# LeCAR-Lab/CoVO-MPC

Hardware: AMD Instinct MI355X
Metric: mpc_control_steps_per_sec (higher is better)
Workload: dtype f32; 1 GPU; covo-online tracking_zigzag N=65536 H=32 lam=0.01 sigma=0.5 (teacher-forced on the recorded inputs -- noisy state, a_mean, key -- of this controller's own 300-step closed-loop episode, timed steps spread evenly over the episode; samples sharded 1x65536, one exchange of the 516-float rank records per step: collective); controller=covo-online, task=tracking_zigzag, N_global=65536, N_local=65536, H=32, pos_stats_info=False

## Files before the change

### covo_mpc_amd/csrc/hessian_adj_body.hpp

```cpp
constexpr int NX = ADJ_NX, NZ = NX + 4, NH = NX + 1, HH = COVO_H, NA = COVO_NA;
constexpr size_t WS_X = 0;
constexpr size_t WS_JF = WS_X + 32 * 16;
constexpr size_t WS_GL = WS_JF + 32 * NX * NZ;
constexpr size_t WS_LAM = WS_GL + 32 * 16;
constexpr size_t WS_MXX = WS_LAM + 33 * 16;
constexpr size_t WS_MXU = WS_MXX + 32 * 256;
constexpr size_t WS_MUU = WS_MXU + 32 * 64;
constexpr size_t WS_S = WS_MUU + 32 * 16;
constexpr int NPAIR = NZ * (NZ + 1) / 2;
constexpr int PAIR_THREADS = (NPAIR + 63) / 64 * 64;
constexpr size_t WS_COUNT = WS_S + (size_t)32 * 16 * NA + 2;
constexpr unsigned long long ADJ_LAM_UNSET = 0xFFF7ADEADBEEF000ull;


__device__ __forceinline__ void adj_force(const float *__restrict__ st, const AdjArgs &A, int bi, int k, double (&f)[3])
{
    if (k == 0) {
        f[0] = st[ST_FDIST + 0]; f[1] = st[ST_FDIST + 1]; f[2] = st[ST_FDIST + 2];
    } else if (A.f_tab != nullptr) {
        const float4 r = A.f_tab[(size_t)bi * HH + k];
        f[0] = r.x; f[1] = r.y; f[2] = r.z;
    } else {
        f[0] = f[1] = f[2] = 0.0;
    }
// ... 363 lines not shown
        const long long t0 = wall_clock64();
        for (;;) {
            bool unset = false;
#pragma unroll
            for (int i = 0; i < NX; ++i) {
                lam[i] = __hip_atomic_load(Lk + i, __ATOMIC_RELAXED, __HIP_MEMORY_SCOPE_AGENT);
                unset |= (unsigned long long)__double_as_longlong(lam[i]) == ADJ_LAM_UNSET;
            }
            if (!unset) break;
            if (wall_clock64() - t0 > 50000000LL) {
                if (A.status != nullptr) __hip_atomic_fetch_or(A.status, COVO_DEVSTAT_ADJOINT, __ATOMIC_RELAXED, __HIP_MEMORY_SCOPE_SYSTEM);
                break;
            }
            __builtin_amdgcn_s_sleep(2);
        }
#pragma unroll
        for (int i = 0; i < NX; ++i) g = fma(lam[i], h[1 + i], g);
    }
    double *__restrict__ Mxx = ws + WS_MXX + (size_t)k * 256, *__restrict__ Mxu = ws + WS_MXU + (size_t)k * 64;
    double *__restrict__ Muu = ws + WS_MUU + (size_t)k * 16;
    if (bb < NX) {
        Mxx[a * 16 + bb] = g;
        Mxx[bb * 16 + a] = g;
    } else if (a < NX) {
        Mxu[a * 4 + (bb - NX)] = g;
    } else {
        Muu[(a - NX) * 4 + (bb - NX)] = g;
        Muu[(bb - NX) * 4 + (a - NX)] = g;
    }
}

__device__ __forceinline__ void adj_hd_padding(const AdjArgs &A, int k, int b, int tid, int nthreads)
{
    double *__restrict__ ws = A.ws + (size_t)b * WS_COUNT;
    double *__restrict__ Mxx = ws + WS_MXX + (size_t)k * 256, *__restrict__ Mxu = ws + WS_MXU + (size_t)k * 64;
    for (int e = tid; e < 256; e += nthreads)
        if ((e >> 4) >= NX || (e & 15) >= NX) Mxx[e] = 0.0;
    if (tid < (16 - NX) * 4) Mxu[NX * 4 + tid] = 0.0;
}

__global__ __launch_bounds__(256) void adj_hd_kernel(const AdjArgs A)
{
    adj_hd_padding(A, (int)blockIdx.x, (int)blockIdx.y, (int)threadIdx.x, 256);
    adj_hd_pairs(A, (int)blockIdx.x, (int)blockIdx.y, (int)threadIdx.x);
}

__global__ __launch_bounds__(256) void adj_chain_kernel(const AdjArgs A)
{
    __shared__ double sjf[(HH - 1) * NX * NZ + 1];
    __shared__ double sgl[HH * 16];
    const int b = blockIdx.y, tid = threadIdx.x, lane = tid & 63, lo = lane & 15, hi = lane >> 4;
    const int w = blockIdx.x;
    double *__restrict__ ws = A.ws + (size_t)b * WS_COUNT;
    if (w >= 9) {
        adj_hd_padding(A, w - 9, b, tid, 256);
        adj_hd_pairs(A, w - 9, b, tid);
        return;
    }
    {
        constexpr int NJ = (HH - 1) * NX * NZ, TJ = (NJ + 255) / 256;
        double vj[TJ];
#pragma unroll
        for (int t = 0; t < TJ; ++t) vj[t] = (tid + 256 * t < NJ) ? ws[WS_JF + tid + 256 * t] : 0.0;
        const double vg0 = ws[WS_GL + tid], vg1 = ws[WS_GL + 256 + tid];
#pragma unroll
        for (int t = 0; t < TJ; ++t)
            if (tid + 256 * t < NJ) sjf[tid + 256 * t] = vj[t];
        sgl[tid] = vg0;
        sgl[256 + tid] = vg1;
        if (tid == 0) sjf[NJ] = 0.0;
    }
    __syncthreads();
    if (tid >= 64) return;
    constexpr int ZI = (HH - 1) * NX * NZ;
    if (w == 8) {
        const double *__restrict__ G = sgl;
        double *__restrict__ L = ws + WS_LAM;
        f64x4 lam;
#pragma unroll
        for (int r = 0; r < 4; ++r) lam[r] = (lo == 0 && hi + 4 * r < NX) ? G[16 * (HH - 1) + hi + 4 * r] : 0.0;
        if (lo == 0) {
#pragma unroll
            for (int r = 0; r < 4; ++r) {
                __hip_atomic_store(&L[16 * (HH - 1) + hi + 4 * r], lam[r], __ATOMIC_RELAXED, __HIP_MEMORY_SCOPE_AGENT);
                __hip_atomic_store(&L[16 * HH + hi + 4 * r], 0.0, __ATOMIC_RELAXED, __HIP_MEMORY_SCOPE_AGENT);
            }
        }
        int offA[4];
        bool okA[4];
#pragma unroll
        for (int g = 0; g < 4; ++g) {
            okA[g] = lo < NX && 4 * g + hi < NX;
            offA[g] = (4 * g + hi) * NZ + lo;
        }
        bool okG[4];
#pragma unroll
        for (int r = 0; r < 4; ++r) okG[r] = lo == 0 && hi + 4 * r < NX;
        double an[4];
        f64x4 gn;
#pragma unroll
        for (int g = 0; g < 4; ++g) an[g] = sjf[okA[g] ? (HH - 2) * NX * NZ + offA[g] : ZI];
#pragma unroll
        for (int r = 0; r < 4; ++r) gn[r] = okG[r] ? G[16 * (HH - 2) + hi + 4 * r] : 0.0;
#pragma unroll
        for (int k = HH - 2; k >= 1; --k) {
            double ac[4];
            f64x4 acc = gn;
#pragma unroll
            for (int g = 0; g < 4; ++g) ac[g] = an[g];
            if (k > 1) {
#pragma unroll
                for (int g = 0; g < 4; ++g) an[g] = sjf[okA[g] ? (k - 1) * NX * NZ + offA[g] : ZI];
#pragma unroll
                for (int r = 0; r < 4; ++r) gn[r] = okG[r] ? G[16 * (k - 1) + hi + 4 * r] : 0.0;
            }
#pragma unroll
            for (int g = 0; g < 4; ++g) acc = __builtin_amdgcn_mfma_f64_16x16x4f64(ac[g], lam[g], acc, 0, 0, 0);
            lam = acc;
            if (lo == 0) {
#pragma unroll
                for (int r = 0; r < 4; ++r) __hip_atomic_store(&L[16 * k + hi + 4 * r], lam[r], __ATOMIC_RELAXED, __HIP_MEMORY_SCOPE_AGENT);
            }
        }
        return;
    }
    const int col = 16 * w + lo, tcol = col >> 2, dcol = col & 3, k0 = 4 * w;
    double *__restrict__ S = ws + WS_S;
    for (int k = 0; k <= k0; ++k) {
#pragma unroll
        for (int r = 0; r < 4; ++r) S[((size_t)k * 16 + hi + 4 * r) * NA + col] = 0.0;
    }
    f64x4 sv = {0.0, 0.0, 0.0, 0.0};
    int offA[4];
    bool okA[4];
#pragma unroll
    for (int g = 0; g < 4; ++g) {
        okA[g] = lo < NX && 4 * g + hi < NX;
        offA[g] = lo * NZ + 4 * g + hi;
    }
    double an[4];
    f64x4 bn;
#pragma unroll
    for (int g = 0; g < 4; ++g) an[g] = sjf[okA[g] ? k0 * NX * NZ + offA[g] : ZI];
#pragma unroll
    for (int r = 0; r < 4; ++r) bn[r] = (tcol == k0 && hi + 4 * r < NX) ? sjf[(k0 * NX + hi + 4 * r) * NZ + NX + dcol] : 0.0;
    double *__restrict__ Sp = S + (size_t)hi * NA + col;
#pragma unroll
    for (int k = 0; k < HH - 1; ++k) {
        if (k < k0) continue;
        double ac[4];
        f64x4 acc = bn;
#pragma unroll
        for (int g = 0; g < 4; ++g) ac[g] = an[g];
        if (k + 1 < HH - 1) {
#pragma unroll
            for (int g = 0; g < 4; ++g) an[g] = sjf[okA[g] ? (k + 1) * NX * NZ + offA[g] : ZI];
            if (k + 1 <= k0 + 3) {
#pragma unroll
                for (int r = 0; r < 4; ++r)
                    bn[r] = (tcol == k + 1 && hi + 4 * r < NX) ? sjf[((k + 1) * NX + hi + 4 * r) * NZ + NX + dcol] : 0.0;
            } else {
#pragma unroll
                for (int r = 0; r < 4; ++r) bn[r] = 0.0;
            }
        }
#pragma unroll
        for (int g = 0; g < 4; ++g) acc = __builtin_amdgcn_mfma_f64_16x16x4f64(ac[g], sv[g], acc, 0, 0, 0);
        sv = acc;
#pragma unroll
        for (int r = 0; r < 4; ++r) Sp[((size_t)(k + 1) * 16 + 4 * r) * NA] = sv[r];
    }
}

__device__ __forceinline__ void adj_tri_tile(int w, int &ti, int &tj)
{
    ti = 0;
    while ((ti + 1) * (ti + 2) / 2 <= w) ++ti;
    tj = w - ti * (ti + 1) / 2;
}

__global__ __launch_bounds__(512) void adj_gemm_kernel(const AdjArgs A)
{
    __shared__ double red[8][4][64];
    __shared__ double sMu[4][64];
    __shared__ double sMuu[64];
    const int b = blockIdx.y, tid = threadIdx.x, lane = tid & 63, wv = tid >> 6, lo = lane & 15, hi = lane >> 4;
    const double *__restrict__ ws = A.ws + (size_t)b * WS_COUNT;
    double *__restrict__ R = A.R + (size_t)b * NA * NA;
    int I, J;
    adj_tri_tile(blockIdx.x, I, J);
    const double *__restrict__ S = ws + WS_S, *__restrict__ Mxx = ws + WS_MXX;
    f64x4 acc = {0.0, 0.0, 0.0, 0.0};
#ifdef KD_PROF
    const long long kp0 = clock64();
#endif
    double ma[4][4], sj[4][4], si[4][4];
#pragma unroll
    for (int it = 0; it < 4; ++it) {
        const int k = 4 * I + 1 + wv + 8 * it;
        const bool on = k < HH;
        const double *__restrict__ Sk = S + (size_t)(on ? k : 0) * 16 * NA, *__restrict__ Mk = Mxx + (size_t)(on ? k : 0) * 256;
        const double2 *__restrict__ Mk2 = reinterpret_cast<const double2 *>(Mk + lo * 16 + 4 * hi);
        const double2 m01 = on ? Mk2[0] : make_double2(0.0, 0.0), m23 = on ? Mk2[1] : make_double2(0.0, 0.0);
        ma[it][0] = m01.x;
        ma[it][1] = m01.y;
        ma[it][2] = m23.x;
        ma[it][3] = m23.y;
#pragma unroll
        for (int g = 0; g < 4; ++g) {
            sj[it][g] = on ? Sk[(size_t)(4 * hi + g) * NA + 16 * J + lo] : 0.0;
            si[it][g] = on ? Sk[(size_t)(4 * g + hi) * NA + 16 * I + lo] : 0.0;
        }
    }
    const int i = 16 * I + hi + 4 * (wv & 3), j = 16 * J + lo;
    const int ti = i >> 2, di = i & 3, tj = j >> 2, dj = j & 3;
    const int tk = ti > tj ? ti : tj, dk = ti > tj ? di : dj;
    double es[NX];
    if (wv < 4) {
        const int col = ti > tj ? j : i;
        const double *__restrict__ Sk = S + (size_t)tk * 16 * NA;
#pragma unroll
        for (int m = 0; m < NX; ++m) es[m] = Sk[(size_t)m * NA + col];
    } else if (wv == 4) {
        sMuu[lane] = ws[WS_MUU + (size_t)(4 * I) * 16 + lane];
    }
// ... 61 lines not shown
```

### covo_mpc_amd/csrc/reduce.hip

```cpp
#include <cstdlib>
#include <cstring>
#include "covo_common.hpp"
#include "softmax_merge.hpp"
#include "softmax_stage1.hpp"

__global__ __launch_bounds__(256) void groupmin_kernel(const float *__restrict__ cost, int N, float *__restrict__ gm)
{
    const int n = blockIdx.x * 256 + threadIdx.x;
    const float wm = wave_min(n < N ? cost[n] : __builtin_inff());
    if ((threadIdx.x & 63) == 0 && (n >> 6) < (N + 63) / 64) gm[n >> 6] = wm;
}


template <bool COV>
__global__ __launch_bounds__(RD_BLOCK) void softmax_partial_kernel(const float *__restrict__ cost,
                                                                   const float4 *__restrict__ a, int N,
                                                                   const float *__restrict__ blockmin, int nbm,
                                                                   float inv_lam, float *__restrict__ partials,
                                                                   const float4 *__restrict__ mu)
{
    softmax_partial_body<COV, false>(cost, a, N, SoftmaxWeights{blockmin, nbm, inv_lam}, partials, mu, nullptr);
}
template <bool COV>
__global__ __launch_bounds__(RD_BLOCK) void softmax_partial_diag_kernel(const float *__restrict__ cost,
                                                                        const float4 *__restrict__ a, int N,
                                                                        const float *__restrict__ blockmin, int nbm,
                                                                        float inv_lam, float *__restrict__ partials,
                                                                        const float4 *__restrict__ mu, float *__restrict__ dpart)
{
    softmax_partial_body<COV, true>(cost, a, N, SoftmaxWeights{blockmin, nbm, inv_lam}, partials, mu, dpart);
}


template <bool FINAL, bool INST = false>
__global__ __launch_bounds__(MG_THREADS) void merge_cov_kernel(const float *__restrict__ partials, int G, float inv_lam,
                                                               const float *__restrict__ a_mean_old, float gamma_mean,
                                                               const float *__restrict__ a_cov_old, float gamma_sigma,
                                                               float *__restrict__ a_mean_out, float *__restrict__ a_cov_out,
                                                               int stride, float *__restrict__ iter_out, int iter_stride)
{
    if (INST) {
        const size_t x = blockIdx.x;
        partials += x * G * stride;
        a_mean_old += x * COVO_NA;
        a_cov_old += x * (COVO_H * 16);
        a_mean_out += x * COVO_NA;
        a_cov_out += x * (COVO_H * 16);
        if (iter_out != nullptr) iter_out += x * (size_t)iter_stride;
    }
    merge_cov_body<FINAL>(partials, G, inv_lam, a_mean_old, gamma_mean, a_cov_old, gamma_sigma, a_mean_out, a_cov_out, stride, iter_out);
}

template <bool FINAL>
__global__ __launch_bounds__(MG_THREADS) void merge_kernel(const float *__restrict__ partials, int G, float inv_lam,
                                                           const float *__restrict__ a_mean_old, float gamma_mean,
                                                           float *__restrict__ out, int stride, float *__restrict__ iter_out,
                                                           int iter_stride)
{
    merge_instance<FINAL, false>(partials, G, inv_lam, a_mean_old, gamma_mean, out, stride, nullptr, nullptr, 0.0f, iter_out, iter_stride);
}

template <bool FINAL>
__global__ __launch_bounds__(MG_THREADS) void merge_diag_kernel(const float *__restrict__ partials, int G, float inv_lam,
                                                                const float *__restrict__ a_mean_old, float gamma_mean,
                                                                float *__restrict__ out, int stride, const float *__restrict__ dpart,
                                                                float *__restrict__ diag_out, float n_samples, float *__restrict__ iter_out,
                                                                int iter_stride)
{
    merge_instance<FINAL, true>(partials, G, inv_lam, a_mean_old, gamma_mean, out, stride, dpart, diag_out, n_samples, iter_out, iter_stride);
}

__global__ void diag_log_rows_kernel(const float *__restrict__ diag, float *__restrict__ log, int n_inst, int stride, int index)
{
    const int i = blockIdx.x * blockDim.x + threadIdx.x;
    if (i < n_inst * COVO_DIAG_FLOATS) {
        const int e = i / COVO_DIAG_FLOATS, j = i % COVO_DIAG_FLOATS;
        log[((size_t)e * stride + index) * COVO_DIAG_FLOATS + j] = diag[i];
    }
}

int launch_diag_log_rows(const float *diag, float *log, int n_inst, int stride, int index, hipStream_t s)
{
    const int n = n_inst * COVO_DIAG_FLOATS;
    hipLaunchKernelGGL(diag_log_rows_kernel, dim3((n + 255) / 256), dim3(256), 0, s, diag, log, n_inst, stride, index);
    COVO_CHECK_HIP(hipGetLastError());
    return 0;
}

__global__ void shift_mean_kernel(const float *__restrict__ in, float *__restrict__ out)
{
    const int i = threadIdx.x;
    out[i] = (i < COVO_NA - COVO_DU) ? in[i + COVO_DU] : in[i];
}

struct Minima {
    const float *blockmin;
    int n_blockmin;
};
static Minima stage1_minima(covo_ctx *h, const UpdateDesc &d, hipStream_t s)
{
    if (d.blockmin != nullptr) return {d.blockmin, d.n_blockmin};
    hipLaunchKernelGGL(groupmin_kernel, dim3((d.N + 255) / 256), dim3(256), 0, s, d.cost, d.N, h->ws_blockmin);
    return {h->ws_blockmin, (d.N + 63) / 64};
}

int launch_softmax_reduce(covo_ctx *h, const UpdateDesc &d, hipStream_t s)
{
    if (d.lam_rows != nullptr) return launch_softmax_reduce_lam(h, d, s);
    const float inv_lam = 1.0f / h->cfg.lam;
    float *partials_ws = d.partials_ws ? d.partials_ws : h->ws_partials;
    const Minima mn = stage1_minima(h, d, s);
    const int grid = stage1_grid(h, d.N);
// ... 97 lines not shown
```

### covo_mpc_amd/csrc/sigma_ns.hip

```cpp
#include "covo_common.hpp"
#include <cstdlib>
#include <cstring>
#include "wave_reduce.hpp"
#include "chol_lds.hpp"
#include "eps_tiles.hpp"
#include "sym_stats.hpp"
#include "noise_gemm_body.hpp"

typedef double f64x4 __attribute__((ext_vector_type(4)));

#ifdef NS_EVAL_STAMPS
#define EV_STAMP(s, i) do { if (threadIdx.x == 0) (s)[SC_STAMPS + 96 + (i)] = (double)wall_clock64(); } while (0)
#else
#define EV_STAMP(s, i) do { } while (0)
#endif
#define EV_STAMP8(s, k, i) do { if ((k) == 8) EV_STAMP(s, 70 + (i)); } while (0)
constexpr int SN = COVO_NA;
constexpr int NS_SQUARINGS = 16;
constexpr double NS_CUT_MARGIN = 1.0 / 1024.0;
constexpr double NS_SQ_TOL = 1e-7;
constexpr double NS_SQ_TGUARD = 1e10;
constexpr int NS_ITERS = 12;
constexpr double NS_TOL2 = 1e-8;
constexpr int RITZ = 4;
// ... 1343 lines not shown
__global__ __launch_bounds__(256) void ns_iter_tail_pair_kernel(const double *A, const NsBufs B, double *scall, int batch, int force_agent)
{
    extern __shared__ __attribute__((aligned(16))) double ld_sm[];
    ns_iter_tail_pair_impl<EARLY_LOGDET>(A, B, scall, batch, force_agent, 0, ld_sm);
}
template <int NEVAL>
__global__ __launch_bounds__(256) void ns_chain_kernel(const double *A, const XBufs xb_all, const NsBufs B, double *scall, int force_agent,
                                                       int deflate)
{
    extern __shared__ __attribute__((aligned(16))) double ld_sm[];
    static_assert(NS_SQ_DYN_DOUBLES * sizeof(double) <= (size_t)SN * (SN + 1) * sizeof(double), "the squaring side's LDS fits the launch's");
    static_assert(NS_SQ_PAIR_WG + NEVAL <= NS_PAIR_WG, "grid = 8 x NS_PAIR_WG covers the squaring side");
    if ((blockIdx.x & 7u) == 0u) {
        ns_square_tail_pair_impl<NEVAL, false, true>(A, xb_all, scall, 1, force_agent, deflate, ld_sm);
        return;
    }
    ns_iter_tail_pair_impl<true>(A, B, scall, 1, force_agent, 1, ld_sm);
}

template <int NWAVES>
__device__ void ns_logdetB_workgroup(const double *__restrict__ A, double *__restrict__ s, double *__restrict__ sm, double *__restrict__ red)
{
    constexpr int THREADS = 64 * NWAVES, LD = SN + 1;
    const int tid = threadIdx.x;
    const double delta = s[SC_DELTA];
    const double2 *A2 = reinterpret_cast<const double2 *>(A);
#pragma unroll 4
    for (int e = tid; e < SN * SN / 2; e += THREADS) {
        const int r = e / (SN / 2), c = 2 * (e % (SN / 2));
        const double2 v = A2[e];
        sm[c * LD + r] = v.x + ((r == c) ? delta : 0.0);
        sm[(c + 1) * LD + r] = v.y + ((r == c + 1) ? delta : 0.0);
    }
    __syncthreads();
    chol128_lds_mfma<LD, NWAVES>(sm, tid);
    if (tid < SN) {
        const double d = sm[tid * LD + tid];
        const double pm = wr::wave64_allprod(__builtin_amdgcn_frexp_mant(d));
        const double pe = wr::wave64_allsum((double)__builtin_amdgcn_frexp_exp(d));
        if ((tid & 63) == 0) {
            red[2 * (tid >> 6)] = pm;
            red[2 * (tid >> 6) + 1] = pe;
        }
    }
    __syncthreads();
    if (tid == 0) {
        const double sumlog = fma(red[1] + red[3], 0.6931471805599453, log(red[0] * red[2]));
        gst<COH_AGENT>(s + SC_SUMLOGB, sumlog);
        asm volatile("s_waitcnt vmcnt(0)" ::: "memory");
        gst<COH_AGENT>(s + SC_LDFLAG, 1.0);
    }
}

__global__ __launch_bounds__(512) void ns_finalize_kernel(const double *__restrict__ Z0all, const double *__restrict__ Z1all,
                                                          const double *__restrict__ Zt0all, const double *__restrict__ Zt1all,
                                                          double *__restrict__ scall, float sample_sigma,
                                                          float *__restrict__ Sigma_out, float *__restrict__ L_out, int batch,
                                                          const EpsGenArgs gen, int *status, const double *__restrict__ Aall,
                                                          int logdet_here)
{
    extern __shared__ __attribute__((aligned(16))) double sm[];
    __shared__ double red[512];
    if (logdet_here && (int)blockIdx.x < 2 * batch && ((int)blockIdx.x & 1) == 0) {
        const int b = (int)blockIdx.x >> 1;
        ns_logdetB_workgroup<8>(Aall + (size_t)b * SN * SN, scall + (size_t)b * SC_COUNT, sm, red);
        return;
    }
    const int first_passenger = logdet_here ? 2 * batch : batch;
    if ((int)blockIdx.x >= first_passenger) {
        eps_tiles_generate(gen, ((int)blockIdx.x - first_passenger) * 8 + (int)(threadIdx.x >> 6), ((int)gridDim.x - first_passenger) * 8,
                           (int)(threadIdx.x & 63));
        return;
    }
    const int b = logdet_here ? (int)blockIdx.x >> 1 : (int)blockIdx.x, tid = threadIdx.x;
    double *s = scall + (size_t)b * SC_COUNT;
    __shared__ double suv[SN];
    const double uv_mine = (tid < SN) ? s[SC_U + tid] : 0.0;
    const bool z1 = s[SC_ZBUF] != 0.0;
    const double zc = s[SC_ZCOEF];
    if (tid < SN) suv[tid] = uv_mine;
    const double *uv = suv;
    const double2 *Z = reinterpret_cast<const double2 *>((z1 ? Z1all : Z0all) + (size_t)b * SN * SN);
    const double2 *Zt = reinterpret_cast<const double2 *>((z1 ? Zt1all : Zt0all) + (size_t)b * SN * SN);
    constexpr int LD = SN + 1;
    const double n = (double)SN;
    long long tk[5];
    tk[0] = clock64();
    {
        constexpr int TR = NS_TILES * 128 / 512;
        double2 za[TR], zt[TR];
#pragma unroll
        for (int t = 0; t < TR; ++t) {
            const int w = __builtin_amdgcn_readfirstlane((tid >> 7) + 4 * t), in = tid & 127;
            int ti, tj;
            tri_tile(w, ti, tj);
            const int e2 = ((16 * ti + (in >> 3)) * SN + 16 * tj + 2 * (in & 7)) >> 1;
            za[t] = Z[e2];
            zt[t] = Zt[e2];
        }
        __syncthreads();
#pragma unroll
        for (int t = 0; t < TR; ++t) {
            const int w = __builtin_amdgcn_readfirstlane((tid >> 7) + 4 * t), in = tid & 127;
            int ti, tj;
            tri_tile(w, ti, tj);
            const int r = 16 * ti + (in >> 3), c = 16 * tj + 2 * (in & 7);
            double v0 = 0.5 * (za[t].x + zt[t].x), v1 = 0.5 * (za[t].y + zt[t].y);
            if (zc != 0.0) {
                const double ur = zc * uv[r];
                v0 = fma(ur, uv[c], v0);
                v1 = fma(ur, uv[c + 1], v1);
            }
            sm[c * LD + r] = v0;
            sm[(c + 1) * LD + r] = v1;
            if (ti == tj) {
                sm[r * LD + c] = v0;
                sm[r * LD + c + 1] = v1;
            }
        }
    }
    __syncthreads();
    tk[1] = clock64();
    chol128_lds_mfma<LD>(sm, tid);
    tk[2] = clock64();
    if (tid == 0) {
        const long long t0 = wall_clock64();
        int good = 1;
        while (gld<COH_AGENT>(s + SC_LDFLAG) == 0.0) {
            __builtin_amdgcn_s_sleep(1);
            if (wall_clock64() - t0 > 20000000LL) {
                good = 0;
                break;
            }
        }
        red[0] = gld<COH_AGENT>(s + SC_SUMLOGB);
        red[1] = good ? 0.0 : 1.0;
    }
    __syncthreads();
    const double sumlogB = red[0];
    const bool ld_failed = red[1] != 0.0;
    const double poison = (s[SC_BARFAIL] != 0.0 || ld_failed) ? __builtin_nan("") : 1.0;
    if (tid == 0 && (s[SC_BARFAIL] != 0.0 || ld_failed) && status != nullptr)
        __hip_atomic_fetch_or(status, COVO_DEVSTAT_GRID_BARRIER, __ATOMIC_RELAXED, __HIP_MEMORY_SCOPE_SYSTEM);
    const double cz = poison * ((double)sample_sigma * (double)sample_sigma) * exp(sumlogB / n) * qm::rsq64_(s[SC_SCALE]);
    const double sq = cz * qm::rsq64_(cz);
    if (tid == 0) s[SC_CZ] = cz;
    tk[3] = clock64();
    constexpr int TRS = SN * SN / 2 / 512;
    double2 za[TRS], zt[TRS];
    if (Sigma_out) {
#pragma unroll
        for (int t = 0; t < TRS; ++t) {
            za[t] = Z[tid + 512 * t];
            zt[t] = Zt[tid + 512 * t];
        }
    }
    float *Lo = L_out + (size_t)b * SN * SN;
#pragma unroll 4
    for (int e = tid; e < SN * SN; e += 512) {
        const int r = e / SN, c = e % SN;
        Lo[e] = (c <= r) ? (float)(sq * sm[c * LD + r]) : 0.0f;
    }
    if (Sigma_out) {
        float2 *So = reinterpret_cast<float2 *>(Sigma_out + (size_t)b * SN * SN);
#pragma unroll
        for (int t = 0; t < TRS; ++t) {
            const int e = 2 * (tid + 512 * t), r = e / SN, c = e % SN;
            double v0 = 0.5 * (za[t].x + zt[t].x), v1 = 0.5 * (za[t].y + zt[t].y);
            if (zc != 0.0) {
                const double ur = zc * uv[r];
                v0 = fma(ur, uv[c], v0);
                v1 = fma(ur, uv[c + 1], v1);
            }
            So[tid + 512 * t] = make_float2((float)(cz * v0), (float)(cz * v1));
        }
    }
    tk[4] = clock64();
    if (tid == 0) {
        for (int i = 0; i < 5; ++i) s[SC_PROF + i] = (double)(tk[i] - tk[0]);
    }
}


struct StreamHook {
    const double *sm;
    double sq;
    float *Lg;
    unsigned *sync;
    unsigned seq;
    int *cnt;
    double *stamps;
    int tid;
    static constexpr int LD = SN + 1;
    __device__ __forceinline__ void panel_done(int p) const
    {
        const int wave = tid >> 6, lane = tid & 63;
#ifdef NS_STREAM_STAMPS
        if (tid == 0) stamps[2 + p] = (double)wall_clock64();
#endif
        if (wave == 0) return;
        const int rr = lane >> 4, kk = lane & 15, j0 = 16 * p, c = j0 + kk;
        for (int i0 = j0 + 4 * (wave - 1); i0 < SN; i0 += 28) {
            const int i = i0 + rr;
            const float v = (c <= i) ? (float)(sq * sm[c * LD + i]) : 0.0f;
            __hip_atomic_store(Lg + (size_t)i * SN + c, v, __ATOMIC_RELAXED, __HIP_MEMORY_SCOPE_AGENT);
        }
    }
    __device__ __forceinline__ void before_barrier(int p) const
    {
        const int wave = tid >> 6, lane = tid & 63;
        if (p == 0 || wave == 0) return;
        asm volatile("s_waitcnt vmcnt(0)" ::: "memory");
        if (lane == 0) {
            const int old = __hip_atomic_fetch_add(cnt + (p - 1), 1, __ATOMIC_RELAXED, __HIP_MEMORY_SCOPE_WORKGROUP);
            if (old == 6) {
                __hip_atomic_store(sync + p, seq, __ATOMIC_RELAXED, __HIP_MEMORY_SCOPE_AGENT);
#ifdef NS_STREAM_STAMPS
                stamps[11 + (p - 1)] = (double)wall_clock64();
#endif
            }
        }
    }
};

template <int P>
__device__ __forceinline__ bool stream_wait_panel(const StreamGemmArgs &S, unsigned seq, int *flag_lds)
{
    if (threadIdx.x == 0) {
        const long long t0 = wall_clock64();
        int good = 1;
        while (__hip_atomic_load(S.sync + 1 + P, __ATOMIC_RELAXED, __HIP_MEMORY_SCOPE_AGENT) != seq) {
            __builtin_amdgcn_s_sleep(1);
            if (wall_clock64() - t0 > 20000000LL) {
                good = 0;
                break;
            }
        }
        *flag_lds = good;
    }
    __syncthreads();
    return *flag_lds != 0;
}
template <int P>
__device__ __forceinline__ void stream_stage_panel(const float *__restrict__ L, float *__restrict__ Ls, int tid)
{
    constexpr int R0 = 32 * (P / 2), CHUNKS = (COVO_NA - R0) * 4;
    if (tid < CHUNKS) {
        const int i = R0 + (tid >> 2), k4 = 16 * P + 4 * (tid & 3);
        const unsigned long long *src = reinterpret_cast<const unsigned long long *>(L + (size_t)i * COVO_NA + k4);
        const unsigned long long lo = __hip_atomic_load(src, __ATOMIC_RELAXED, __HIP_MEMORY_SCOPE_AGENT);
        const unsigned long long hi = __hip_atomic_load(src + 1, __ATOMIC_RELAXED, __HIP_MEMORY_SCOPE_AGENT);
        float *d = Ls + i * NG_LDA + k4;
        d[0] = (k4 + 0 <= i) ? __uint_as_float((unsigned)lo) : 0.0f;
        d[1] = (k4 + 1 <= i) ? __uint_as_float((unsigned)(lo >> 32)) : 0.0f;
        d[2] = (k4 + 2 <= i) ? __uint_as_float((unsigned)hi) : 0.0f;
        d[3] = (k4 + 3 <= i) ? __uint_as_float((unsigned)(hi >> 32)) : 0.0f;
    }
}
__global__ __launch_bounds__(512) void ns_finalize_stream_kernel(const double *__restrict__ Z0, const double *__restrict__ Z1,
                                                                 const double *__restrict__ Zt0, const double *__restrict__ Zt1,
                                                                 double *__restrict__ s, float sample_sigma, const StreamGemmArgs S,
                                                                 int *status)
{
    extern __shared__ __attribute__((aligned(16))) double sm[];
    __shared__ double red[8];
    __shared__ int flag_lds;
    const int tid = threadIdx.x, lane = tid & 63;
    const int wave = __builtin_amdgcn_readfirstlane(tid >> 6);
    constexpr int LD = SN + 1;
    const double n = (double)SN;
    if (tid == 0) {
        const long long t0 = wall_clock64();
        int good = 1;
        while (gld<COH_AGENT>(s + SC_LDFLAG) == 0.0) {
            __builtin_amdgcn_s_sleep(1);
            if (wall_clock64() - t0 > 20000000LL) {
                good = 0;
                break;
            }
        }
        red[0] = gld<COH_AGENT>(s + SC_SUMLOGB);
        red[1] = good ? 0.0 : 1.0;
    }
    __syncthreads();
    const double sumlogB = red[0];
    const bool bad = s[SC_BARFAIL] != 0.0 || red[1] != 0.0;
    const double poison = bad ? __builtin_nan("") : 1.0;
    const double cz = poison * ((double)sample_sigma * (double)sample_sigma) * exp(sumlogB / n) * qm::rsq64_(s[SC_SCALE]);
    const double sq = cz * qm::rsq64_(cz);
    const unsigned seq = __hip_atomic_load(S.sync, __ATOMIC_RELAXED, __HIP_MEMORY_SCOPE_AGENT);
    const bool z1 = s[SC_ZBUF] != 0.0;
    const double zc = s[SC_ZCOEF];
#ifdef NS_STREAM_STAMPS
    double *stamps = s + SC_STAMPS;
#define STREAM_STAMP(i) do { if (tid == 0) stamps[(i)] = (double)wall_clock64(); } while (0)
#else
#define STREAM_STAMP(i) do { } while (0)
#endif

    if (blockIdx.x == 0) {
        STREAM_STAMP(0);
        if (tid == 0 && bad && status != nullptr)
            __hip_atomic_fetch_or(status, COVO_DEVSTAT_GRID_BARRIER, __ATOMIC_RELAXED, __HIP_MEMORY_SCOPE_SYSTEM);
        if (tid == 0) s[SC_CZ] = cz;
        __shared__ double suv[SN];
        __shared__ int wcnt[8];
        if (tid < SN) suv[tid] = s[SC_U + tid];
        if (tid < 8) wcnt[tid] = 0;
        const double2 *Z = reinterpret_cast<const double2 *>(z1 ? Z1 : Z0);
        const double2 *Zt = reinterpret_cast<const double2 *>(z1 ? Zt1 : Zt0);
        long long tk[3];
        tk[0] = clock64();
        {
            constexpr int TR = NS_TILES * 128 / 512;
            double2 za[TR], zt[TR];
#pragma unroll
            for (int t = 0; t < TR; ++t) {
                const int w = __builtin_amdgcn_readfirstlane((tid >> 7) + 4 * t), in = tid & 127;
                int ti, tj;
                tri_tile(w, ti, tj);
                const int e2 = ((16 * ti + (in >> 3)) * SN + 16 * tj + 2 * (in & 7)) >> 1;
                za[t] = Z[e2];
                zt[t] = Zt[e2];
            }
            __syncthreads();
#pragma unroll
            for (int t = 0; t < TR; ++t) {
                const int w = __builtin_amdgcn_readfirstlane((tid >> 7) + 4 * t), in = tid & 127;
                int ti, tj;
                tri_tile(w, ti, tj);
                const int r = 16 * ti + (in >> 3), c = 16 * tj + 2 * (in & 7);
                double v0 = 0.5 * (za[t].x + zt[t].x), v1 = 0.5 * (za[t].y + zt[t].y);
                if (zc != 0.0) {
                    const double ur = zc * suv[r];
                    v0 = fma(ur, suv[c], v0);
                    v1 = fma(ur, suv[c + 1], v1);
                }
                sm[c * LD + r] = v0;
                sm[(c + 1) * LD + r] = v1;
                if (ti == tj) {
                    sm[r * LD + c] = v0;
                    sm[r * LD + c + 1] = v1;
                }
            }
        }
        __syncthreads();
        tk[1] = clock64();
        STREAM_STAMP(1);
        StreamHook hook;
        hook.sm = sm;
        hook.sq = sq;
        hook.Lg = S.L_stream;
        hook.sync = S.sync;
        hook.seq = seq;
        hook.cnt = wcnt;
#ifdef NS_STREAM_STAMPS
        hook.stamps = stamps;
#else
        hook.stamps = nullptr;
#endif
        hook.tid = tid;
        chol128_lds_mfma<LD, 8>(sm, tid, hook);
        hook.before_barrier(8);
        tk[2] = clock64();
        if (tid == 0) {
#ifdef NS_STREAM_STAMPS
            stamps[10] = (double)wall_clock64();
#endif
            for (int i = 0; i < 3; ++i) s[SC_PROF + i] = (double)(tk[i] - tk[0]);
        }
        return;
    }

    float *Ls = reinterpret_cast<float *>(sm);
    float *mus = Ls + COVO_NA * NG_LDA;
    float4 *epsx = reinterpret_cast<float4 *>(mus + COVO_NA);
    const int b = (int)blockIdx.x, W = (int)gridDim.x - 1;
#ifdef NS_STREAM_STAMPS
    double *wst = (tid == 0 && (b == 1 || b == W)) ? stamps + (b == 1 ? 24 : 56) : nullptr;
#else
    double *const wst = nullptr;
#endif
    if (wst) wst[0] = (double)wall_clock64();
    if (tid < COVO_NA) mus[tid] = S.mu[tid];
    const uint32_t k0 = S.dyn[0], k1 = S.dyn[1];
    const int N = S.N, ntiles = (N + 31) / 32;
    const int nextra = ntiles < 8 ? ntiles : 8;
    const int j = lane & 31, kh = lane >> 5;
    const int t0 = 8 * b + wave;
    const bool has0 = t0 < ntiles;
    int ex = -1;
    if (W >= 64) { if ((b & 7) == 0 && (b >> 3) - 1 < nextra) ex = (b >> 3) - 1; }
    else if (b - 1 < nextra) ex = b - 1;
    auto id_of = [&](int t) {
        int row = t * 32 + j;
        row = row < N ? row : N - 1;
        return (uint64_t)(S.sample_offset + row);
    };
    const uint64_t id0 = id_of(has0 ? t0 : 0);
    BGroup bq[4];
    if (has0) {
#pragma unroll
        for (int g = 0; g < 4; ++g) bq[g] = gen_group(id0, g, kh, k0, k1);
    }
    if (ex >= 0) {
        const uint64_t idx = id_of(ex);
#pragma unroll
        for (int q = 2 * wave; q < 2 * wave + 2; ++q) epsx[q * 64 + lane] = rngd::normal4((uint32_t)(2 * q + kh), idx, k0, k1);
    }
    const int xrole = ex >= 0 ? wave : 0;
    if (S.a_cov_out != nullptr && b - 1 < SN * SN / 512) {
        const double *Zb = z1 ? Z1 : Z0, *Ztb = z1 ? Zt1 : Zt0;
        const int wstride = W < SN * SN / 512 ? W : SN * SN / 512;
        for (int e = (b - 1) * 512 + tid; e < SN * SN; e += wstride * 512) {
            double v = 0.5 * (Zb[e] + Ztb[e]);
            if (zc != 0.0) v = fma(zc * s[SC_U + e / SN], s[SC_U + e % SN], v);
            S.a_cov_out[e] = (float)(cz * v);
        }
    }
    f32x16 acc0[4], accx[4];
#pragma unroll
    for (int rt = 0; rt < 4; ++rt)
#pragma unroll
        for (int e = 0; e < 16; ++e) { acc0[rt][e] = 0.0f; accx[rt][e] = 0.0f; }
    const float *__restrict__ La = Ls + j * NG_LDA + kh;
    float4 *__restrict__ a_out = reinterpret_cast<float4 *>(S.a_out);
    bool ok = true;
    auto store_rt = [&](int rt, int tile, const f32x16 (&acc)[4]) {
        const int nn = tile * 32 + j;
        if (nn < N) {
#pragma unroll
            for (int g = 0; g < 4; ++g) {
                const int t = 8 * rt + 2 * g + kh;
                const float4 m4 = *reinterpret_cast<const float4 *>(mus + 4 * t);
                float4 v;
                if (S.nanp) {
                    v.x = qm::clip11_nan_(m4.x + acc[rt][4 * g + 0]);
                    v.y = qm::clip11_nan_(m4.y + acc[rt][4 * g + 1]);
                    v.z = qm::clip11_nan_(m4.z + acc[rt][4 * g + 2]);
                    v.w = qm::clip11_nan_(m4.w + acc[rt][4 * g + 3]);
                } else {
                    v.x = qm::clip11_(m4.x + acc[rt][4 * g + 0]);
                    v.y = qm::clip11_(m4.y + acc[rt][4 * g + 1]);
                    v.z = qm::clip11_(m4.z + acc[rt][4 * g + 2]);
                    v.w = qm::clip11_(m4.w + acc[rt][4 * g + 3]);
                }
                if (!ok) v = make_float4(__builtin_nanf(""), __builtin_nanf(""), __builtin_nanf(""), __builtin_nanf(""));
                a_out[(size_t)t * N + nn] = v;
            }
        }
    };
    auto xgroup = [&](int g) {
        BGroup bx;
#pragma unroll
        for (int i = 0; i < 4; ++i) bx.c[i] = epsx[(4 * g + i) * 64 + lane];
        return bx;
    };
#define STREAM_PANEL(P)                                                                                           \
    do {                                                                                                          \
        constexpr int G_ = (P) / 2, H_ = (P) & 1;                                                                 \
        ok = stream_wait_panel<P>(S, seq, &flag_lds) && ok;                                                       \
        if (wst) wst[1 + 3 * (P)] = (double)wall_clock64();                                                       \
        stream_stage_panel<P>(S.L_stream, Ls, tid);                                                               \
        __syncthreads();                                                                                          \
        if (wst) wst[2 + 3 * (P)] = (double)wall_clock64();                                                       \
        if (has0) mfma_half<G_, H_, 15>(La, bq[G_], acc0);                                                        \
        if (xrole == 1) mfma_half<G_, H_, 8>(La, xgroup(G_), accx);                                               \
        else if (xrole == 2) mfma_half<G_, H_, 4>(La, xgroup(G_), accx);                                          \
        else if (xrole == 3) mfma_half<G_, H_, 3>(La, xgroup(G_), accx);                                          \
        if (H_ == 1) {                                                                                            \
            if (has0) store_rt(G_, t0, acc0);                                                                     \
            if ((G_ == 3 && xrole == 1) || (G_ == 2 && xrole == 2) || (G_ < 2 && xrole == 3)) store_rt(G_, ex, accx); \
        }                                                                                                         \
        if (wst) wst[3 + 3 * (P)] = (double)wall_clock64();                                                       \
    } while (0)
    STREAM_PANEL(0);
    STREAM_PANEL(1);
    STREAM_PANEL(2);
    STREAM_PANEL(3);
    STREAM_PANEL(4);
    STREAM_PANEL(5);
    STREAM_PANEL(6);
    STREAM_PANEL(7);
#undef STREAM_PANEL
    if (!ok && S.a_cov_out != nullptr && b - 1 < SN * SN / 512) {
        const int wstride = W < SN * SN / 512 ? W : SN * SN / 512;
        for (int e = (b - 1) * 512 + tid; e < SN * SN; e += wstride * 512) S.a_cov_out[e] = __builtin_nanf("");
    }
    if (!ok && tid == 0 && status != nullptr)
        __hip_atomic_fetch_or(status, COVO_DEVSTAT_GRID_BARRIER, __ATOMIC_RELAXED, __HIP_MEMORY_SCOPE_SYSTEM);
}

SymStatsOut sigma_ns_stats_out(void *workspace, int batch)
{
    double *ws = reinterpret_cast<double *>(workspace);
    double *sc = ws + (size_t)11 * batch * SN * SN;
    SymStatsOut o;
    o.rpart = sc + SC_RPART;
    o.fpart = sc + SC_FPART;
    o.diag = sc + SC_DIAG;
    o.stride = SC_COUNT;
    o.flags = sc + SC_FLAGS;
    o.ready = sc + SC_READY;
    return o;
}
size_t sigma_ns_workspace_bytes(int batch) { return (size_t)batch * ((11 + NS_SQUARINGS - 1) * SN * SN + SC_COUNT) * sizeof(double); }

template <int MI, int MJ>
static void ns_launch_iters(hipStream_t s, const NsBufs &B, double *sc, int i_end, int batch)
{
    hipLaunchKernelGGL(ns_first_elem_kernel, ns_grid(65, batch), dim3(256), 0, s, B.A, B.X1, B.Y[1], B.Yt[1], B.Z[1], B.Zt[1], sc, 1, batch);
    for (int i = 1; i < i_end; ++i) {
        const int in = i & 1, out = in ^ 1;
        hipLaunchKernelGGL((ns_T_quad_kernel<MI, MJ>), ns_grid(64 / (MI * MJ), batch), dim3(256), 0, s, B.Y[in], B.Zt[in], B.T, B.Tt, sc, i,
                           batch);
        hipLaunchKernelGGL((ns_YZ_quad_kernel<MI, MJ>), ns_grid(128 / (MI * MJ), batch), dim3(256), 0, s, B.Yt[in], B.Z[in], B.T, B.Tt,
                           B.Y[out], B.Yt[out], B.Z[out], B.Zt[out], sc, i, out, batch);
    }
}

int launch_sigma_ns(const CovoOpts &opt, const SigmaNsDesc &d, void *workspace, hipStream_t s, const DebugMasks &dbg)
{
    const double *R = d.R;
    const int batch = d.batch;
    const float sample_sigma = d.sample_sigma;
    float *Sigma = d.Sigma;
    CovDeferred *cov = d.cov;
    const StreamGemmArgs *stream = d.stream;
    const int sigma_stages = dbg.sigma_stages;
    if (d.streamed != nullptr) *d.streamed = false;
    double *ws = reinterpret_cast<double *>(workspace);
    const size_t M = (size_t)batch * SN * SN;
    double *A = ws;
    double *Y[2] = {ws + 3 * M, ws + 4 * M}, *Yt[2] = {ws + 5 * M, ws + 6 * M};
    double *Z[2] = {ws + 7 * M, ws + 8 * M}, *Zt[2] = {ws + 9 * M, ws + 10 * M};
    double *sc = ws + 11 * M;
    double *hist0 = sc + (size_t)batch * SC_COUNT;
    const XBufs xb{ws + M, ws + 2 * M, hist0, hist0 + (size_t)(NS_SQUARINGS - 2) * M, M};
// ... 118 lines not shown
```

Before: 6158 control-steps/s.

## Defer logdet flag wait off the streaming kernel's critical entry path

Result: faster. 6241 control-steps/s (median of 6 runs) (+1.3%).

```diff
diff --git a/covo_mpc_amd/csrc/hessian_adj_body.hpp b/covo_mpc_amd/csrc/hessian_adj_body.hpp
--- a/covo_mpc_amd/csrc/hessian_adj_body.hpp
+++ b/covo_mpc_amd/csrc/hessian_adj_body.hpp
@@ -439,6 +439,9 @@
     const int b = blockIdx.y, tid = threadIdx.x, lane = tid & 63, lo = lane & 15, hi = lane >> 4;
     const int w = blockIdx.x;
     double *__restrict__ ws = A.ws + (size_t)b * WS_COUNT;
+#ifdef KC_STAMPS
+    const long long kc0 = wall_clock64();
+#endif
     if (w >= 9) {
         adj_hd_padding(A, w - 9, b, tid, 256);
         adj_hd_pairs(A, w - 9, b, tid);
@@ -457,7 +460,21 @@
         sgl[256 + tid] = vg1;
         if (tid == 0) sjf[NJ] = 0.0;
     }
+#ifdef KC_STAMPS
+    const long long kc1 = wall_clock64();
+#endif
     __syncthreads();
+#ifdef KC_STAMPS
+    const long long kc2 = wall_clock64();
+#define KC_STAMP_END()                                                                                                       \
+    do {                                                                                                                     \
+        if (tid == 0 && b == 0 && (w == 0 || w == 7 || w == 8))                                                              \
+            printf("KC wg %d: filled %lld first-mfma %lld end %lld (10 ns ticks from entry)\n", w, kc1 - kc0, kc2 - kc0,      \
+                   (long long)wall_clock64() - kc0);                                                                         \
+    } while (0)
+#else
+#define KC_STAMP_END() do { } while (0)
+#endif
     if (tid >= 64) return;
     constexpr int ZI = (HH - 1) * NX * NZ;
     if (w == 8) {
@@ -509,6 +526,7 @@
                 for (int r = 0; r < 4; ++r) __hip_atomic_store(&L[16 * k + hi + 4 * r], lam[r], __ATOMIC_RELAXED, __HIP_MEMORY_SCOPE_AGENT);
             }
         }
+        KC_STAMP_END();
         return;
     }
     const int col = 16 * w + lo, tcol = col >> 2, dcol = col & 3, k0 = 4 * w;
@@ -557,7 +575,9 @@
 #pragma unroll
         for (int r = 0; r < 4; ++r) Sp[((size_t)(k + 1) * 16 + 4 * r) * NA] = sv[r];
     }
-}
+    KC_STAMP_END();
+}
+#undef KC_STAMP_END
 
 __device__ __forceinline__ void adj_tri_tile(int w, int &ti, int &tj)
 {
diff --git a/covo_mpc_amd/csrc/reduce.hip b/covo_mpc_amd/csrc/reduce.hip
--- a/covo_mpc_amd/csrc/reduce.hip
+++ b/covo_mpc_amd/csrc/reduce.hip
@@ -57,7 +57,23 @@
                                                            float *__restrict__ out, int stride, float *__restrict__ iter_out,
                                                            int iter_stride)
 {
+#ifdef MERGE_STAMPS
+    const long long mt0 = wall_clock64();
+    float touch = 0.0f;
+    {
+        const float *p = partials + (size_t)blockIdx.x * G * stride;
+        const int col = threadIdx.x & (COVO_NA - 1), slice = threadIdx.x >> 7;
+        for (int g = slice; g < G; g += MG_SLICES) touch += p[(size_t)g * stride + 2 + col];
+        if ((int)threadIdx.x < G) touch += p[(size_t)threadIdx.x * stride] + p[(size_t)threadIdx.x * stride + 1];
+    }
+    asm volatile("s_waitcnt vmcnt(0)" : "+v"(touch)::"memory");
+    const long long mt1 = wall_clock64();
+#endif
     merge_instance<FINAL, false>(partials, G, inv_lam, a_mean_old, gamma_mean, out, stride, nullptr, nullptr, 0.0f, iter_out, iter_stride);
+#ifdef MERGE_STAMPS
+    if (threadIdx.x == 0 && blockIdx.x == 0)
+        printf("merge G %d: records-in-hand %lld done %lld (10 ns ticks from entry)\n", G, mt1 - mt0, (long long)wall_clock64() - mt0);
+#endif
 }
 
 template <bool FINAL>
diff --git a/covo_mpc_amd/csrc/sigma_ns.hip b/covo_mpc_amd/csrc/sigma_ns.hip
--- a/covo_mpc_amd/csrc/sigma_ns.hip
+++ b/covo_mpc_amd/csrc/sigma_ns.hip
@@ -1419,6 +1419,40 @@
     }
 }
 
+__device__ __forceinline__ void ns_logdet_fence() { asm volatile("" ::: "memory"); }
+__device__ __forceinline__ bool ns_logdet_timed_out(const double *s, double flag)
+{
+    const long long t0 = wall_clock64();
+    bool timed_out = false;
+    while (flag == 0.0) {
+        __builtin_amdgcn_s_sleep(1);
+        if (wall_clock64() - t0 > 20000000LL) {
+            timed_out = true;
+            break;
+        }
+        flag = gld<COH_AGENT>(s + SC_LDFLAG);
+    }
+    ns_logdet_fence();
+    return timed_out;
+}
+__device__ __forceinline__ double ns_cz(bool bad, float sample_sigma, double sumlogB, double scale)
+{
+    const double poison = bad ? __builtin_nan("") : 1.0;
+    return poison * ((double)sample_sigma * (double)sample_sigma) * exp(sumlogB / (double)SN) * qm::rsq64_(scale);
+}
+__device__ __forceinline__ void tri_tile_panel0_first(int round, int g, int &ti, int &tj)
+{
+    if (round < 2) {
+        ti = 4 * round + g;
+        tj = 0;
+    } else {
+        const int k = 4 * (round - 2) + g;
+        const int t7 = (k >= 1) + (k >= 3) + (k >= 6) + (k >= 10) + (k >= 15) + (k >= 21);
+        ti = t7 + 1;
+        tj = k - t7 * (t7 + 1) / 2 + 1;
+    }
+}
+
 __global__ __launch_bounds__(512) void ns_finalize_kernel(const double *__restrict__ Z0all, const double *__restrict__ Z1all,
                                                           const double *__restrict__ Zt0all, const double *__restrict__ Zt1all,
                                                           double *__restrict__ scall, float sample_sigma,
@@ -1445,12 +1479,12 @@
     const double uv_mine = (tid < SN) ? s[SC_U + tid] : 0.0;
     const bool z1 = s[SC_ZBUF] != 0.0;
     const double zc = s[SC_ZCOEF];
+    const double barfail = s[SC_BARFAIL], scale = s[SC_SCALE];
     if (tid < SN) suv[tid] = uv_mine;
     const double *uv = suv;
     const double2 *Z = reinterpret_cast<const double2 *>((z1 ? Z1all : Z0all) + (size_t)b * SN * SN);
     const double2 *Zt = reinterpret_cast<const double2 *>((z1 ? Zt1all : Zt0all) + (size_t)b * SN * SN);
     constexpr int LD = SN + 1;
-    const double n = (double)SN;
     long long tk[5];
     tk[0] = clock64();
     {
@@ -1491,25 +1525,15 @@
     chol128_lds_mfma<LD>(sm, tid);
     tk[2] = clock64();
     if (tid == 0) {
-        const long long t0 = wall_clock64();
-        int good = 1;
-        while (gld<COH_AGENT>(s + SC_LDFLAG) == 0.0) {
-            __builtin_amdgcn_s_sleep(1);
-            if (wall_clock64() - t0 > 20000000LL) {
-                good = 0;
-                break;
-            }
-        }
+        const bool timed_out = ns_logdet_timed_out(s, gld<COH_AGENT>(s + SC_LDFLAG));
         red[0] = gld<COH_AGENT>(s + SC_SUMLOGB);
-        red[1] = good ? 0.0 : 1.0;
-    }
-    __syncthreads();
-    const double sumlogB = red[0];
-    const bool ld_failed = red[1] != 0.0;
-    const double poison = (s[SC_BARFAIL] != 0.0 || ld_failed) ? __builtin_nan("") : 1.0;
-    if (tid == 0 && (s[SC_BARFAIL] != 0.0 || ld_failed) && status != nullptr)
+        red[1] = timed_out ? 1.0 : 0.0;
+    }
+    __syncthreads();
+    const bool bad = barfail != 0.0 || red[1] != 0.0;
+    if (tid == 0 && bad && status != nullptr)
         __hip_atomic_fetch_or(status, COVO_DEVSTAT_GRID_BARRIER, __ATOMIC_RELAXED, __HIP_MEMORY_SCOPE_SYSTEM);
-    const double cz = poison * ((double)sample_sigma * (double)sample_sigma) * exp(sumlogB / n) * qm::rsq64_(s[SC_SCALE]);
+    const double cz = ns_cz(bad, sample_sigma, red[0], scale);
     const double sq = cz * qm::rsq64_(cz);
     if (tid == 0) s[SC_CZ] = cz;
     tk[3] = clock64();
@@ -1551,7 +1575,12 @@
 
 struct StreamHook {
     const double *sm;
-    double sq;
+    double *s;
+    double *czq;
+    double sumlogB, barfail, scale;
+    bool ld_timed_out;
+    float sample_sigma;
+    int *status;
     float *Lg;
     unsigned *sync;
     unsigned seq;
@@ -1559,6 +1588,17 @@
     double *stamps;
     int tid;
     static constexpr int LD = SN + 1;
+    static constexpr int CZ_TID = 64;
+    __device__ __forceinline__ void form_cz() const
+    {
+        const bool bad = barfail != 0.0 || ld_timed_out;
+        if (bad && status != nullptr)
+            __hip_atomic_fetch_or(status, COVO_DEVSTAT_GRID_BARRIER, __ATOMIC_RELAXED, __HIP_MEMORY_SCOPE_SYSTEM);
+        const double cz = ns_cz(bad, sample_sigma, sumlogB, scale);
+        czq[0] = cz;
+        czq[1] = cz * qm::rsq64_(cz);
+        s[SC_CZ] = cz;
+    }
     __device__ __forceinline__ void panel_done(int p) const
     {
         const int wave = tid >> 6, lane = tid & 63;
@@ -1566,6 +1606,7 @@
         if (tid == 0) stamps[2 + p] = (double)wall_clock64();
 #endif
         if (wave == 0) return;
+        const double sq = czq[1];
         const int rr = lane >> 4, kk = lane & 15, j0 = 16 * p, c = j0 + kk;
         for (int i0 = j0 + 4 * (wave - 1); i0 < SN; i0 += 28) {
             const int i = i0 + rr;
@@ -1576,6 +1617,7 @@
     __device__ __forceinline__ void before_barrier(int p) const
     {
         const int wave = tid >> 6, lane = tid & 63;
+        if (p == 0 && tid == CZ_TID) form_cz();
         if (p == 0 || wave == 0) return;
         asm volatile("s_waitcnt vmcnt(0)" ::: "memory");
         if (lane == 0) {
@@ -1635,29 +1677,6 @@
     const int tid = threadIdx.x, lane = tid & 63;
     const int wave = __builtin_amdgcn_readfirstlane(tid >> 6);
     constexpr int LD = SN + 1;
-    const double n = (double)SN;
-    if (tid == 0) {
-        const long long t0 = wall_clock64();
-        int good = 1;
-        while (gld<COH_AGENT>(s + SC_LDFLAG) == 0.0) {
-            __builtin_amdgcn_s_sleep(1);
-            if (wall_clock64() - t0 > 20000000LL) {
-                good = 0;
-                break;
-            }
-        }
-        red[0] = gld<COH_AGENT>(s + SC_SUMLOGB);
-        red[1] = good ? 0.0 : 1.0;
-    }
-    __syncthreads();
-    const double sumlogB = red[0];
-    const bool bad = s[SC_BARFAIL] != 0.0 || red[1] != 0.0;
-    const double poison = bad ? __builtin_nan("") : 1.0;
-    const double cz = poison * ((double)sample_sigma * (double)sample_sigma) * exp(sumlogB / n) * qm::rsq64_(s[SC_SCALE]);
-    const double sq = cz * qm::rsq64_(cz);
-    const unsigned seq = __hip_atomic_load(S.sync, __ATOMIC_RELAXED, __HIP_MEMORY_SCOPE_AGENT);
-    const bool z1 = s[SC_ZBUF] != 0.0;
-    const double zc = s[SC_ZCOEF];
 #ifdef NS_STREAM_STAMPS
     double *stamps = s + SC_STAMPS;
 #define STREAM_STAMP(i) do { if (tid == 0) stamps[(i)] = (double)wall_clock64(); } while (0)
@@ -1667,35 +1686,43 @@
 
     if (blockIdx.x == 0) {
         STREAM_STAMP(0);
-        if (tid == 0 && bad && status != nullptr)
-            __hip_atomic_fetch_or(status, COVO_DEVSTAT_GRID_BARRIER, __ATOMIC_RELAXED, __HIP_MEMORY_SCOPE_SYSTEM);
-        if (tid == 0) s[SC_CZ] = cz;
+        const bool z1 = s[SC_ZBUF] != 0.0;
+        const double zc = s[SC_ZCOEF];
+        const double ldflag = gld<COH_AGENT>(s + SC_LDFLAG);
+        const double barfail = s[SC_BARFAIL], scale = s[SC_SCALE];
+        const double uv_mine = (tid < SN) ? s[SC_U + tid] : 0.0;
+        const unsigned seq = __hip_atomic_load(S.sync, __ATOMIC_RELAXED, __HIP_MEMORY_SCOPE_AGENT);
         __shared__ double suv[SN];
         __shared__ int wcnt[8];
-        if (tid < SN) suv[tid] = s[SC_U + tid];
-        if (tid < 8) wcnt[tid] = 0;
         const double2 *Z = reinterpret_cast<const double2 *>(z1 ? Z1 : Z0);
         const double2 *Zt = reinterpret_cast<const double2 *>(z1 ? Zt1 : Zt0);
         long long tk[3];
         tk[0] = clock64();
+        StreamHook hook;
+        hook.ld_timed_out = false;
         {
             constexpr int TR = NS_TILES * 128 / 512;
             double2 za[TR], zt[TR];
 #pragma unroll
             for (int t = 0; t < TR; ++t) {
-                const int w = __builtin_amdgcn_readfirstlane((tid >> 7) + 4 * t), in = tid & 127;
+                const int g = __builtin_amdgcn_readfirstlane(tid >> 7), in = tid & 127;
                 int ti, tj;
-                tri_tile(w, ti, tj);
+                tri_tile_panel0_first(t, g, ti, tj);
                 const int e2 = ((16 * ti + (in >> 3)) * SN + 16 * tj + 2 * (in & 7)) >> 1;
                 za[t] = Z[e2];
                 zt[t] = Zt[e2];
             }
-            __syncthreads();
+            if (tid < SN) suv[tid] = uv_mine;
+            if (tid < 8) wcnt[tid] = 0;
+            if (tid == StreamHook::CZ_TID) hook.ld_timed_out = ns_logdet_timed_out(s, ldflag);
+            ns_logdet_fence();
+            hook.sumlogB = gld<COH_AGENT>(s + SC_SUMLOGB);
+            if (zc != 0.0) __syncthreads();
 #pragma unroll
             for (int t = 0; t < TR; ++t) {
-                const int w = __builtin_amdgcn_readfirstlane((tid >> 7) + 4 * t), in = tid & 127;
+                const int g = __builtin_amdgcn_readfirstlane(tid >> 7), in = tid & 127;
                 int ti, tj;
-                tri_tile(w, ti, tj);
+                tri_tile_panel0_first(t, g, ti, tj);
                 const int r = 16 * ti + (in >> 3), c = 16 * tj + 2 * (in & 7);
                 double v0 = 0.5 * (za[t].x + zt[t].x), v1 = 0.5 * (za[t].y + zt[t].y);
                 if (zc != 0.0) {
@@ -1711,12 +1738,18 @@
                 }
             }
         }
+        tk[1] = clock64();
+#ifdef NS_STREAM_STAMPS
         __syncthreads();
-        tk[1] = clock64();
+#endif
         STREAM_STAMP(1);
-        StreamHook hook;
         hook.sm = sm;
-        hook.sq = sq;
+        hook.s = s;
+        hook.czq = red;
+        hook.barfail = barfail;
+        hook.scale = scale;
+        hook.sample_sigma = sample_sigma;
+        hook.status = status;
         hook.Lg = S.L_stream;
         hook.sync = S.sync;
         hook.seq = seq;
@@ -1743,6 +1776,17 @@
     float *mus = Ls + COVO_NA * NG_LDA;
     float4 *epsx = reinterpret_cast<float4 *>(mus + COVO_NA);
     const int b = (int)blockIdx.x, W = (int)gridDim.x - 1;
+    const unsigned seq = __hip_atomic_load(S.sync, __ATOMIC_RELAXED, __HIP_MEMORY_SCOPE_AGENT);
+    const bool cov_writer = S.a_cov_out != nullptr && b - 1 < SN * SN / 512;
+    bool z1 = false;
+    double zc = 0.0, ldflag = 0.0, barfail = 0.0, scale = 0.0;
+    if (cov_writer) {
+        z1 = s[SC_ZBUF] != 0.0;
+        zc = s[SC_ZCOEF];
+        ldflag = gld<COH_AGENT>(s + SC_LDFLAG);
+        barfail = s[SC_BARFAIL];
+        scale = s[SC_SCALE];
+    }
 #ifdef NS_STREAM_STAMPS
     double *wst = (tid == 0 && (b == 1 || b == W)) ? stamps + (b == 1 ? 24 : 56) : nullptr;
 #else
@@ -1776,7 +1820,14 @@
         for (int q = 2 * wave; q < 2 * wave + 2; ++q) epsx[q * 64 + lane] = rngd::normal4((uint32_t)(2 * q + kh), idx, k0, k1);
     }
     const int xrole = ex >= 0 ? wave : 0;
-    if (S.a_cov_out != nullptr && b - 1 < SN * SN / 512) {
+    if (cov_writer) {
+        if (tid == 0) {
+            const bool timed_out = ns_logdet_timed_out(s, ldflag);
+            red[0] = gld<COH_AGENT>(s + SC_SUMLOGB);
+            red[1] = timed_out ? 1.0 : 0.0;
+        }
+        __syncthreads();
+        const double cz = ns_cz(barfail != 0.0 || red[1] != 0.0, sample_sigma, red[0], scale);
         const double *Zb = z1 ? Z1 : Z0, *Ztb = z1 ? Zt1 : Zt0;
         const int wstride = W < SN * SN / 512 ? W : SN * SN / 512;
         for (int e = (b - 1) * 512 + tid; e < SN * SN; e += wstride * 512) {
@@ -1850,7 +1901,7 @@
     STREAM_PANEL(6);
     STREAM_PANEL(7);
 #undef STREAM_PANEL
-    if (!ok && S.a_cov_out != nullptr && b - 1 < SN * SN / 512) {
+    if (!ok && cov_writer) {
         const int wstride = W < SN * SN / 512 ? W : SN * SN / 512;
         for (int e = (b - 1) * 512 + tid; e < SN * SN; e += wstride * 512) S.a_cov_out[e] = __builtin_nanf("");
     }
```
